# MoayedHajiAli/ElasticDiffusion-official

Measured on AMD Instinct MI355X. Metric: images/sec at 50 steps (SDXL 2048x1024), higher is better.
Workload: dtype fp16

## Files before the change

### elasticdiffusion_official_amd/csrc/gemm_kernels.hip

```cpp
#include <hip/hip_runtime.h>
#include <stdint.h>
#include <stdlib.h>

#include "elastic_hip.h"

namespace {

typedef float f32x4 __attribute__((ext_vector_type(4)));
typedef __bf16 bf16x8 __attribute__((ext_vector_type(8)));
typedef _Float16 f16x8 __attribute__((ext_vector_type(8)));
typedef uint32_t u32x4 __attribute__((ext_vector_type(4)));
typedef __attribute__((address_space(3))) void* lds_ptr_t;

struct BF {
  typedef bf16x8 v8;
  static __device__ __forceinline__ f32x4 mfma(v8 a, v8 b, f32x4 c) {
    return __builtin_amdgcn_mfma_f32_16x16x32_bf16(a, b, c, 0, 0, 0);
  }
  static __device__ __forceinline__ float to_f32(uint16_t h) { return __builtin_bit_cast(float, (uint32_t)h << 16); }
  static __device__ __forceinline__ uint16_t from_f32(float f) { return __builtin_bit_cast(uint16_t, (__bf16)f); }
  static __device__ __forceinline__ uint32_t pack2(float lo, float hi) {
    typedef float f2 __attribute__((ext_vector_type(2)));
    typedef __bf16 b2 __attribute__((ext_vector_type(2)));
    return __builtin_bit_cast(uint32_t, __builtin_convertvector(f2{lo, hi}, b2));
  }
};
struct HF {
  typedef f16x8 v8;
  static __device__ __forceinline__ f32x4 mfma(v8 a, v8 b, f32x4 c) {
    return __builtin_amdgcn_mfma_f32_16x16x32_f16(a, b, c, 0, 0, 0);
  }
  static __device__ __forceinline__ float to_f32(uint16_t h) { return (float)__builtin_bit_cast(_Float16, h); }
  static __device__ __forceinline__ uint16_t from_f32(float f) { return __builtin_bit_cast(uint16_t, (_Float16)f); }
  static __device__ __forceinline__ uint32_t pack2(float lo, float hi) {
    typedef float f2 __attribute__((ext_vector_type(2)));
    typedef _Float16 h2 __attribute__((ext_vector_type(2)));
    return __builtin_bit_cast(uint32_t, __builtin_convertvector(f2{lo, hi}, h2));
  }
};

constexpr int BM = 256;
constexpr int BN = 128;
constexpr int BK = 64;
constexpr int SUB = 1024;
constexpr int W_REGION = 32768;
constexpr int BUF = 65536;

__device__ __forceinline__ int swz(int p) { return p ^ (((p >> 9) & 1) << 5); }
__device__ __forceinline__ constexpr int x_sub(int rg, int kh) { return (rg * 2 + kh) * SUB; }
__device__ __forceinline__ constexpr int w_sub(int rg, int kh) { return W_REGION + (rg * 2 + kh) * SUB; }

__device__ __forceinline__ float gelu_as(float x) {
  const float z = __builtin_fabsf(x) * 0.70710678118654752f;
  const float t = __builtin_amdgcn_rcpf(__builtin_fmaf(0.3275911f, z, 1.0f));
  float p = __builtin_fmaf(1.061405429f, t, -1.453152027f);
  p = __builtin_fmaf(p, t, 1.421413741f);
  p = __builtin_fmaf(p, t, -0.284496736f);
  p = __builtin_fmaf(p, t, 0.254829592f);
  const float q = p * t * __builtin_amdgcn_exp2f(-1.4426950408889634f * z * z);
  const float h = 0.5f * x * q;
  return x > 0.f ? x - h : h;
}

__device__ __forceinline__ float abs_mul(float a, float b) {
  float r;
  asm("v_mul_f32_e64 %0, |%1|, %2" : "=v"(r) : "v"(a), "v"(b));
  return r;
}
__device__ __forceinline__ float relu1(float a) {
  float r;
  asm("v_max_f32_e32 %0, 0, %1" : "=v"(r) : "v"(a));
  return r;
}
__device__ __forceinline__ float geglu_one(float v, float g) {
  const float z = abs_mul(g, 0.70710678118654752f);
  const float t = __builtin_amdgcn_rcpf(__builtin_fmaf(0.3275911f, z, 1.0f));
  float p = __builtin_fmaf(0.5f * 1.061405429f, t, 0.5f * -1.453152027f);
  p = __builtin_fmaf(p, t, 0.5f * 1.421413741f);
  p = __builtin_fmaf(p, t, 0.5f * -0.284496736f);
  p = __builtin_fmaf(p, t, 0.5f * 0.254829592f);
  const float hq = (p * t) * __builtin_amdgcn_exp2f((-1.4426950408889634f * z) * z);
  return v * (relu1(g) - abs_mul(g, hq));
}

#define ED_WAIT_VM(n) asm volatile("s_waitcnt vmcnt(" #n ")" ::: "memory")
#define ED_WAIT_LGKM(n) asm volatile("s_waitcnt lgkmcnt(" #n ")" ::: "memory")
#define ED_BARRIER()                          \
  do {                                        \
    asm volatile("s_barrier" ::: "memory");   \
    __builtin_amdgcn_sched_barrier(0);        \
  } while (0)

struct Ctx {
  __amdgpu_buffer_rsrc_t xr, wr_;
  int x_voff[2], w_voff[2];
  int px_mask[2];
  int img_w, cin2, cpt;
  int wave;
  int xrd, wrd;
};

constexpr int CONV_UP2X = 2;
constexpr int CONV_S2 = 3;
constexpr int CONV_S2P0 = 4;
struct KPos {
  int tile, tap, ct, w;
};
template <int CONV>
__device__ __forceinline__ KPos k_next(KPos p, int cpt) {
  ++p.tile;
  if (CONV) {
    ++p.tap;
    p.w += cpt;
    if (p.tap == 9) {
      p.tap = 0;
      ++p.ct;
      p.w = p.ct;
    }
  } else {
    p.w = p.tile;
  }
  return p;
}

template <int BUFI, int CONV>
__device__ __forceinline__ void stage_x(uint8_t* lds, const Ctx& c, KPos p, int h) {
  const int rg = (c.wave & 3) + 8 * (c.wave >> 2) + 4 * h;
  uint8_t* dst = lds + BUFI * BUF + x_sub(0, 0) + rg * (2 * SUB);
  if (CONV) {
    const int dy = p.tap / 3 - 1, dx = p.tap - 3 * (p.tap / 3) - 1;
    int delta;
    if (CONV == CONV_UP2X) {
      const int yp = (c.px_mask[h] >> 16) & 1, xp = (c.px_mask[h] >> 17) & 1;
      delta = (((yp + dy) >> 1) * c.img_w + ((xp + dx) >> 1)) * c.cin2 + p.ct * (BK * 2);
    } else {
      delta = (dy * c.img_w + dx) * c.cin2 + p.ct * (BK * 2);
    }
    const int vo = ((c.px_mask[h] >> p.tap) & 1) ? c.x_voff[h] + delta : (int)0x80000000;
    __builtin_amdgcn_raw_ptr_buffer_load_lds(c.xr, (lds_ptr_t)dst, 16, vo, 0, 0, 0);
    __builtin_amdgcn_raw_ptr_buffer_load_lds(c.xr, (lds_ptr_t)(dst + SUB), 16, vo + 64, 0, 0, 0);
  } else {
    const int vo = c.x_voff[h] + p.tile * (BK * 2);
    __builtin_amdgcn_raw_ptr_buffer_load_lds(c.xr, (lds_ptr_t)dst, 16, vo, 0, 0, 0);
    __builtin_amdgcn_raw_ptr_buffer_load_lds(c.xr, (lds_ptr_t)(dst + SUB), 16, vo + 64, 0, 0, 0);
  }
}
template <int BUFI>
__device__ __forceinline__ void stage_w(uint8_t* lds, const Ctx& c, int widx, int g) {
  const int rg = 8 * g + c.wave;
  const int vo = c.w_voff[g] + widx * (BK * 2);
  uint8_t* dst = lds + BUFI * BUF + w_sub(0, 0) + rg * (2 * SUB);
  __builtin_amdgcn_raw_ptr_buffer_load_lds(c.wr_, (lds_ptr_t)dst, 16, vo, 0, 0, 0);
  __builtin_amdgcn_raw_ptr_buffer_load_lds(c.wr_, (lds_ptr_t)(dst + SUB), 16, vo + 64, 0, 0, 0);
}

template <class T>
struct Frags {
  typename T::v8 x[4][2];
  typename T::v8 wv[2][2];
  typename T::v8 wg[2][2];
};

template <class T, int BUFI>
__device__ __forceinline__ void read_x(const uint8_t* lds, const Ctx& c, Frags<T>& f, int mh) {
#pragma unroll
  for (int mf = 0; mf < 4; ++mf)
#pragma unroll
    for (int kh = 0; kh < 2; ++kh)
      f.x[mf][kh] = *reinterpret_cast<const typename T::v8*>(lds + c.xrd + BUFI * BUF + x_sub(mh * 4 + mf, kh));
}
template <class T, int BUFI, int G>
__device__ __forceinline__ void read_w(const uint8_t* lds, const Ctx& c, Frags<T>& f) {
#pragma unroll
  for (int nf = 0; nf < 2; ++nf)
#pragma unroll
    for (int kh = 0; kh < 2; ++kh) {
      typename T::v8 v = *reinterpret_cast<const typename T::v8*>(lds + c.wrd + BUFI * BUF + w_sub(8 * G + nf, kh) - W_REGION);
      if (G == 0) f.wv[nf][kh] = v; else f.wg[nf][kh] = v;
    }
}

template <class T, int MH, int G>
__device__ __forceinline__ void mma16(f32x4 (&acc)[8][4], const Frags<T>& f) {
  __builtin_amdgcn_s_setprio(1);
#pragma unroll
  for (int kh = 0; kh < 2; ++kh)
#pragma unroll
    for (int mf = 0; mf < 4; ++mf)
#pragma unroll
      for (int nf = 0; nf < 2; ++nf)
        acc[MH * 4 + mf][G * 2 + nf] = T::mfma(G == 0 ? f.wv[nf][kh] : f.wg[nf][kh], f.x[mf][kh], acc[MH * 4 + mf][G * 2 + nf]);
  __builtin_amdgcn_s_setprio(0);
}

template <class T, int BUFI, int CONV, bool FIRST = false>
__device__ __forceinline__ void tile_phases(uint8_t* lds, const Ctx& c, Frags<T>& f, f32x4 (&acc)[8][4], int tile, bool s1,
                                            bool s2, KPos p1, KPos p2) {
  read_w<T, BUFI, 0>(lds, c, f);
  __builtin_amdgcn_sched_barrier(0);
  read_x<T, BUFI>(lds, c, f, 0);
  if (s1) stage_x<BUFI ^ 1, CONV>(lds, c, p1, 1);
  ED_WAIT_LGKM(8);
  if (FIRST) ED_WAIT_VM(10);
  ED_BARRIER();
  ED_WAIT_LGKM(0);
  __builtin_amdgcn_sched_barrier(0);
  mma16<T, 0, 0>(acc, f);
  if (FIRST) ED_WAIT_VM(10);
  ED_BARRIER();
  read_w<T, BUFI, 1>(lds, c, f);
  if (s2) stage_w<BUFI>(lds, c, p2.w, 0);
  if (FIRST) ED_WAIT_VM(10);
  ED_BARRIER();
  ED_WAIT_LGKM(0);
  __builtin_amdgcn_sched_barrier(0);
  mma16<T, 0, 1>(acc, f);
  if (FIRST) ED_WAIT_VM(10);
  ED_BARRIER();
  read_x<T, BUFI>(lds, c, f, 1);
  if (s2) stage_x<BUFI, CONV>(lds, c, p2, 0);
  ED_BARRIER();
  ED_WAIT_LGKM(0);
  __builtin_amdgcn_sched_barrier(0);
  mma16<T, 1, 1>(acc, f);
  ED_BARRIER();
  if (s2) {
    stage_w<BUFI>(lds, c, p2.w, 1);
    ED_WAIT_VM(6);
  } else {
    ED_WAIT_VM(0);
  }
  ED_BARRIER();
  mma16<T, 1, 0>(acc, f);
  ED_BARRIER();
}

constexpr int TWO_MIN_TILES = 20;
template <class T, int BUFI, int CONV>
__device__ __forceinline__ void tile_phases_two(uint8_t* lds, const Ctx& c, Frags<T>& f, f32x4 (&acc)[8][4], int tile, bool s1, bool s2,
                                                KPos p1, KPos p2) {
  read_w<T, BUFI, 0>(lds, c, f);
  read_x<T, BUFI>(lds, c, f, 0);
  read_w<T, BUFI, 1>(lds, c, f);
  if (s1) stage_x<BUFI ^ 1, CONV>(lds, c, p1, 1);
  ED_WAIT_LGKM(0);
  ED_BARRIER();
  mma16<T, 0, 0>(acc, f);
  mma16<T, 0, 1>(acc, f);
  ED_BARRIER();
  read_x<T, BUFI>(lds, c, f, 1);
  if (s2) {
    stage_w<BUFI>(lds, c, p2.w, 0);
    stage_x<BUFI, CONV>(lds, c, p2, 0);
    stage_w<BUFI>(lds, c, p2.w, 1);
    ED_WAIT_VM(6);
  } else {
    ED_WAIT_VM(0);
  }
  ED_WAIT_LGKM(0);
  ED_BARRIER();
  mma16<T, 1, 1>(acc, f);
  mma16<T, 1, 0>(acc, f);
  ED_BARRIER();
}

template <class T, int BUFI, int CONV>
__device__ __forceinline__ void tile_phases_half(uint8_t* lds, const Ctx& c, Frags<T>& f, f32x4 (&acc)[8][4], int tile, bool s1, bool s2,
                                                 KPos p1, KPos p2) {
  read_w<T, BUFI, 0>(lds, c, f);
  read_x<T, BUFI>(lds, c, f, 0);
  if (s1) stage_x<BUFI ^ 1, CONV>(lds, c, p1, 1);
  ED_WAIT_LGKM(0);
  ED_BARRIER();
  mma16<T, 0, 0>(acc, f);
  ED_BARRIER();
  read_x<T, BUFI>(lds, c, f, 1);
  if (s2) {
    stage_w<BUFI>(lds, c, p2.w, 0);
    stage_x<BUFI, CONV>(lds, c, p2, 0);
    ED_WAIT_VM(4);
  } else {
    ED_WAIT_VM(0);
  }
  ED_WAIT_LGKM(0);
  ED_BARRIER();
  mma16<T, 1, 0>(acc, f);
  ED_BARRIER();
}

template <class T, int BUFI, int CONV>
__device__ __forceinline__ void tile_phases_rows(uint8_t* lds, const Ctx& c, Frags<T>& f, f32x4 (&acc)[8][4], bool s1, bool s2, KPos p1,
                                                 KPos p2) {
  read_w<T, BUFI, 0>(lds, c, f);
  read_x<T, BUFI>(lds, c, f, 0);
  if (s1) stage_w<BUFI ^ 1>(lds, c, p1.w, 1);
  ED_WAIT_LGKM(0);
  ED_BARRIER();
  mma16<T, 0, 0>(acc, f);
  ED_BARRIER();
  read_w<T, BUFI, 1>(lds, c, f);
  if (s2) {
    stage_w<BUFI>(lds, c, p2.w, 0);
    stage_x<BUFI, CONV>(lds, c, p2, 0);
    ED_WAIT_VM(4);
  } else {
    ED_WAIT_VM(0);
  }
  ED_WAIT_LGKM(0);
  ED_BARRIER();
  mma16<T, 0, 1>(acc, f);
  ED_BARRIER();
}

template <class T, int EPI, int CONV, bool ADD = true, bool OUT32 = false, bool TWO = false, bool ROWS = false>
__global__ void __launch_bounds__(512, 2)
k_gemm_8phase(const uint16_t* __restrict__ x, const uint16_t* __restrict__ w, const uint16_t* __restrict__ bias,
              const uint16_t* __restrict__ row_bias, const uint16_t* __restrict__ residual, uint16_t* __restrict__ out, int M,
              int K, int I, int n_blocks_n, int n_blocks, int img_h, int img_w, int rows_per_sample, float out_scale,
              const float* __restrict__ act_absmax) {
  __shared__ __attribute__((aligned(1024))) uint8_t lds[2 * BUF];

  const int bid = blockIdx.x;
  const int q = n_blocks >> 3, r = n_blocks & 7, xcd = bid & 7;
  const int tid = (xcd < r ? xcd * (q + 1) : r * (q + 1) + (xcd - r) * q) + (bid >> 3);
  const int n_blocks_m = n_blocks / n_blocks_n;
  const int per_group = 8 * n_blocks_n, grp = tid / per_group, first = grp * 8;
  const int rows_here = n_blocks_m - first < 8 ? n_blocks_m - first : 8;
  constexpr int TBM = ROWS ? BM / 2 : BM;
  constexpr int WROWS = TBM / 2;
  constexpr int NMB = WROWS / 16;
  const int m0 = (first + (tid % per_group) % rows_here) * TBM;
  const int n0 = ((tid % per_group) / rows_here) * (EPI == 0 ? BN : 2 * BN);
  const int gap = EPI == 0 ? I : BN;

  const int lane = threadIdx.x & 63;
  Ctx c;
  c.wave = __builtin_amdgcn_readfirstlane(threadIdx.x >> 6);
  const int wrow = c.wave >> 2, wcol = c.wave & 3;

  const int ps = swz(16 * lane), srow = ps >> 6, skb = ps & 63;
  const int row_bytes = K * 2;
  const int x_row_bytes = CONV ? row_bytes / 9 : row_bytes;
  c.xr = __builtin_amdgcn_make_buffer_rsrc((void*)x, 0, (int)((int64_t)(CONV == CONV_UP2X ? M / 4 : CONV >= CONV_S2 ? 4 * (int64_t)M : M) * x_row_bytes),
                                           0x00020000);
  c.wr_ = __builtin_amdgcn_make_buffer_rsrc((void*)w, 0, (int)((int64_t)(EPI == 0 ? 2 : 1) * I * row_bytes), 0x00020000);
  const int xrow0 = m0 + ((c.wave & 3) + (ROWS ? 4 : 8) * (c.wave >> 2)) * 16 + srow;
  c.x_voff[0] = xrow0 * x_row_bytes + skb;
  c.x_voff[1] = c.x_voff[0] + 64 * x_row_bytes;
  c.img_w = CONV == CONV_UP2X ? img_w / 2 : CONV >= CONV_S2 ? 2 * img_w : img_w;
  c.cin2 = x_row_bytes;
  c.cpt = CONV ? K / (9 * BK) : 1;
  c.px_mask[0] = c.px_mask[1] = 0;
  if (CONV) {
#pragma unroll
    for (int h = 0; h < 2; ++h) {
      const int m = xrow0 + 64 * h;
      if (m < M) {
        const int rem = m % (img_h * img_w), py = rem / img_w, px = rem - py * img_w;
        int mask = 0;
#pragma unroll
        for (int t = 0; t < 9; ++t) {
          if (CONV == CONV_S2) {
            if (2 * py + t / 3 - 1 >= 0 && 2 * px + t % 3 - 1 >= 0) mask |= 1 << t;
          } else if (CONV == CONV_S2P0) {
            if (2 * py + t / 3 < 2 * img_h && 2 * px + t % 3 < 2 * img_w) mask |= 1 << t;
          } else {
            const int yy = py + t / 3 - 1, xx = px + t % 3 - 1;
            if (yy >= 0 && yy < img_h && xx >= 0 && xx < img_w) mask |= 1 << t;
          }
        }
        c.px_mask[h] = mask;
        if (CONV == CONV_UP2X) {
          const int hs = img_h / 2, ws = img_w / 2;
          c.px_mask[h] = mask | ((py & 1) << 16) | ((px & 1) << 17);
          c.x_voff[h] = ((m / (img_h * img_w)) * (hs * ws) + (py >> 1) * ws + (px >> 1)) * x_row_bytes + skb;
        }
        if (CONV >= CONV_S2) {
          const int o1 = CONV == CONV_S2P0 ? 1 : 0;
          c.x_voff[h] = (((m / (img_h * img_w)) * (2 * img_h) + 2 * py + o1) * (2 * img_w) + 2 * px + o1) * x_row_bytes + skb;
        }
      }
    }
  }
  c.w_voff[0] = (n0 + 32 * (c.wave >> 1) + 8 * (srow >> 2) + (srow & 3) + 4 * (c.wave & 1)) * row_bytes + skb;
  c.w_voff[1] = c.w_voff[0] + gap * row_bytes;
  const int rd = swz((lane & 15) * 64 + (lane >> 4) * 16);
  c.xrd = rd + wrow * 8 * (2 * SUB);
  c.wrd = rd + W_REGION + wcol * 2 * (2 * SUB);

  const int ncol = n0 + 32 * wcol + 8 * (lane >> 4);
  u32x4 bias_v = {0, 0, 0, 0}, bias_g = {0, 0, 0, 0};
  if (bias && !OUT32) {
    if (EPI == 0 || ncol < I) bias_v = *reinterpret_cast<const u32x4*>(bias + ncol);
    if (EPI == 0 || ncol + gap < I) bias_g = *reinterpret_cast<const u32x4*>(bias + gap + ncol);
  }

  f32x4 acc[8][4];
#pragma unroll
  for (int a = 0; a < 8; ++a)
#pragma unroll
    for (int b = 0; b < 4; ++b) acc[a][b] = f32x4{0.f, 0.f, 0.f, 0.f};
  Frags<T> f;

  const int nt = K / BK;
  const KPos p0 = {0, 0, 0, 0};
  KPos pa = k_next<CONV>(p0, c.cpt);
  KPos pb = k_next<CONV>(pa, c.cpt);
  const bool half = !ROWS && EPI == 1 && n0 + BN >= I;
  if (ROWS) {
    stage_w<0>(lds, c, 0, 0);
    stage_x<0, CONV>(lds, c, p0, 0);
    stage_w<0>(lds, c, 0, 1);
    if (nt > 1) {
      stage_w<1>(lds, c, pa.w, 0);
      stage_x<1, CONV>(lds, c, pa, 0);
      ED_WAIT_VM(4);
    } else {
      ED_WAIT_VM(0);
    }
    ED_BARRIER();
    if (wrow == 1) ED_BARRIER();
    int tr = 0;
    for (; tr + 1 < nt; tr += 2) {
      tile_phases_rows<T, 0, CONV>(lds, c, f, acc, true, tr + 2 < nt, pa, pb);
      pa = pb;
      pb = k_next<CONV>(pb, c.cpt);
      tile_phases_rows<T, 1, CONV>(lds, c, f, acc, tr + 2 < nt, tr + 3 < nt, pa, pb);
      pa = pb;
      pb = k_next<CONV>(pb, c.cpt);
    }
    if (tr < nt) tile_phases_rows<T, 0, CONV>(lds, c, f, acc, false, false, pa, pb);
    if (wrow == 0) ED_BARRIER();
  } else if (half) {
    stage_w<0>(lds, c, 0, 0);
    stage_x<0, CONV>(lds, c, p0, 0);
    stage_x<0, CONV>(lds, c, p0, 1);
    if (nt > 1) {
      stage_w<1>(lds, c, pa.w, 0);
      stage_x<1, CONV>(lds, c, pa, 0);
      ED_WAIT_VM(4);
    } else {
      ED_WAIT_VM(0);
    }
    ED_BARRIER();
    if (wrow == 1) ED_BARRIER();
    int th = 0;
    for (; th + 1 < nt; th += 2) {
      tile_phases_half<T, 0, CONV>(lds, c, f, acc, th, true, th + 2 < nt, pa, pb);
      pa = pb;
      pb = k_next<CONV>(pb, c.cpt);
      tile_phases_half<T, 1, CONV>(lds, c, f, acc, th + 1, th + 2 < nt, th + 3 < nt, pa, pb);
      pa = pb;
      pb = k_next<CONV>(pb, c.cpt);
    }
    if (th < nt) tile_phases_half<T, 0, CONV>(lds, c, f, acc, th, false, false, pa, pb);
    if (wrow == 0) ED_BARRIER();
  } else {
  stage_w<0>(lds, c, 0, 0);
  stage_x<0, CONV>(lds, c, p0, 0);
  stage_w<0>(lds, c, 0, 1);
  stage_x<0, CONV>(lds, c, p0, 1);
  constexpr bool two = TWO;
  const bool early = nt >= 3 && !two;
  if (nt > 1) {
    stage_w<1>(lds, c, pa.w, 0);
    stage_x<1, CONV>(lds, c, pa, 0);
    stage_w<1>(lds, c, pa.w, 1);
    if (early) ED_WAIT_VM(10);
    else ED_WAIT_VM(6);
  } else {
    ED_WAIT_VM(0);
  }
  ED_BARRIER();
  if (wrow == 1) ED_BARRIER();

  int t = 0;
  if (two) {
    for (; t + 1 < nt; t += 2) {
      tile_phases_two<T, 0, CONV>(lds, c, f, acc, t, true, t + 2 < nt, pa, pb);
      pa = pb;
      pb = k_next<CONV>(pb, c.cpt);
      tile_phases_two<T, 1, CONV>(lds, c, f, acc, t + 1, t + 2 < nt, t + 3 < nt, pa, pb);
      pa = pb;
      pb = k_next<CONV>(pb, c.cpt);
    }
    if (t < nt) tile_phases_two<T, 0, CONV>(lds, c, f, acc, t, false, false, pa, pb);
    t = nt;
  }
  if (early) {
    tile_phases<T, 0, CONV, true>(lds, c, f, acc, 0, true, true, pa, pb);
    pa = pb;
    pb = k_next<CONV>(pb, c.cpt);
    tile_phases<T, 1, CONV>(lds, c, f, acc, 1, true, 3 < nt, pa, pb);
    pa = pb;
    pb = k_next<CONV>(pb, c.cpt);
    t = 2;
  }
  for (; t + 1 < nt; t += 2) {
    tile_phases<T, 0, CONV>(lds, c, f, acc, t, true, t + 2 < nt, pa, pb);
    pa = pb;
    pb = k_next<CONV>(pb, c.cpt);
    tile_phases<T, 1, CONV>(lds, c, f, acc, t + 1, t + 2 < nt, t + 3 < nt, pa, pb);
    pa = pb;
    pb = k_next<CONV>(pb, c.cpt);
  }
  if (t < nt) tile_phases<T, 0, CONV>(lds, c, f, acc, t, false, false, pa, pb);
  if (wrow == 0) ED_BARRIER();
  }

  if (OUT32) {
    const float* biasf = reinterpret_cast<const float*>(bias);
    const float* resf = reinterpret_cast<const float*>(residual);
    float* outf = reinterpret_cast<float*>(out);
    if (act_absmax) {
      const int E = (int)((__builtin_bit_cast(uint32_t, *act_absmax) >> 23) & 0xffu) - 127;
      const int e = E > 14 ? E - 14 : 0;
      out_scale *= __builtin_bit_cast(float, (uint32_t)(127 + e) << 23);
    }
    const bool col_v = ncol < I, col_g = ncol + gap < I;
    f32x4 b32[2][2] = {{f32x4{0.f, 0.f, 0.f, 0.f}, f32x4{0.f, 0.f, 0.f, 0.f}}, {f32x4{0.f, 0.f, 0.f, 0.f}, f32x4{0.f, 0.f, 0.f, 0.f}}};
    if (biasf) {
#pragma unroll
      for (int fr = 0; fr < 2; ++fr) {
        if (col_v) b32[0][fr] = *reinterpret_cast<const f32x4*>(biasf + ncol + 4 * fr);
        if (col_g) b32[1][fr] = *reinterpret_cast<const f32x4*>(biasf + ncol + gap + 4 * fr);
      }
    }
#pragma unroll
    for (int mb = 0; mb < NMB; ++mb) {
      const int m = m0 + WROWS * wrow + 16 * mb + (lane & 15);
      if (m >= M) continue;
#pragma unroll
      for (int hf = 0; hf < 2; ++hf) {
        if (!(hf == 0 ? col_v : col_g)) continue;
        const int64_t o = (int64_t)m * I + ncol + hf * gap;
#pragma unroll
        for (int fr = 0; fr < 2; ++fr) {
          f32x4 v = acc[mb][2 * hf + fr] * out_scale + b32[hf][fr];
          if (ADD && resf) v += *reinterpret_cast<const f32x4*>(resf + o + 4 * fr);
          *reinterpret_cast<f32x4*>(outf + o + 4 * fr) = v;
        }
      }
    }
    return;
  }
  float bv[2][4], bg[2][4];
#pragma unroll
  for (int e = 0; e < 8; ++e) {
    bv[e >> 2][e & 3] = T::to_f32((uint16_t)(bias_v[e >> 1] >> (16 * (e & 1))));
    bg[e >> 2][e & 3] = T::to_f32((uint16_t)(bias_g[e >> 1] >> (16 * (e & 1))));
  }
#pragma unroll
  for (int mb = 0; mb < NMB; ++mb) {
    const int m = m0 + WROWS * wrow + 16 * mb + (lane & 15);
    if (EPI == 0) {
      uint32_t pk[4];
#pragma unroll
      for (int nf = 0; nf < 2; ++nf)
#pragma unroll
        for (int jj = 0; jj < 2; ++jj) {
          const float o0 = geglu_one(acc[mb][nf][2 * jj] + bv[nf][2 * jj], acc[mb][2 + nf][2 * jj] + bg[nf][2 * jj]);
          const float o1 = geglu_one(acc[mb][nf][2 * jj + 1] + bv[nf][2 * jj + 1], acc[mb][2 + nf][2 * jj + 1] + bg[nf][2 * jj + 1]);
          pk[nf * 2 + jj] = T::pack2(o0, o1);
        }
      if (m < M) *reinterpret_cast<u32x4*>(out + (int64_t)m * I + ncol) = u32x4{pk[0], pk[1], pk[2], pk[3]};
    } else {
      const bool ok_v = m < M && ncol < I, ok_g = m < M && ncol + gap < I;
      u32x4 av[2] = {u32x4{0, 0, 0, 0}, u32x4{0, 0, 0, 0}}, ag[2] = {u32x4{0, 0, 0, 0}, u32x4{0, 0, 0, 0}};
      if (ADD && row_bias) {
        const int64_t rb = (int64_t)(m / rows_per_sample) * I;
        if (ok_v) av[0] = *reinterpret_cast<const u32x4*>(row_bias + rb + ncol);
        if (ok_g) ag[0] = *reinterpret_cast<const u32x4*>(row_bias + rb + ncol + gap);
      }
      if (ADD && residual) {
        if (ok_v) av[1] = *reinterpret_cast<const u32x4*>(residual + (int64_t)m * I + ncol);
        if (ok_g) ag[1] = *reinterpret_cast<const u32x4*>(residual + (int64_t)m * I + ncol + gap);
      }
      uint32_t pv[4], pg[4];
#pragma unroll
      for (int e = 0; e < 8; e += 2) {
        float v0 = acc[mb][e >> 2][e & 3] + bv[e >> 2][e & 3], v1 = acc[mb][e >> 2][(e & 3) + 1] + bv[e >> 2][(e & 3) + 1];
        float g0 = acc[mb][2 + (e >> 2)][e & 3] + bg[e >> 2][e & 3], g1 = acc[mb][2 + (e >> 2)][(e & 3) + 1] + bg[e >> 2][(e & 3) + 1];
        if (ADD) {
#pragma unroll
          for (int a = 0; a < 2; ++a) {
            v0 += T::to_f32((uint16_t)av[a][e >> 1]), v1 += T::to_f32((uint16_t)(av[a][e >> 1] >> 16));
            g0 += T::to_f32((uint16_t)ag[a][e >> 1]), g1 += T::to_f32((uint16_t)(ag[a][e >> 1] >> 16));
          }
        }
        pv[e >> 1] = (uint32_t)T::from_f32(v0) | ((uint32_t)T::from_f32(v1) << 16);
        pg[e >> 1] = (uint32_t)T::from_f32(g0) | ((uint32_t)T::from_f32(g1) << 16);
      }
      if (ok_v) *reinterpret_cast<u32x4*>(out + (int64_t)m * I + ncol) = u32x4{pv[0], pv[1], pv[2], pv[3]};
      if (ok_g) *reinterpret_cast<u32x4*>(out + (int64_t)m * I + ncol + gap) = u32x4{pg[0], pg[1], pg[2], pg[3]};
    }
  }
}

struct TilePos {
  int m0, n0;
};
__device__ __forceinline__ TilePos geglu_tile_of(int bid, int n_blocks, int n_blocks_n) {
  const int q = n_blocks >> 3, r = n_blocks & 7, xcd = bid & 7;
  const int tid = (xcd < r ? xcd * (q + 1) : r * (q + 1) + (xcd - r) * q) + (bid >> 3);
  const int n_blocks_m = n_blocks / n_blocks_n;
  const int per_group = 8 * n_blocks_n, grp = tid / per_group, first = grp * 8;
  const int rows_here = n_blocks_m - first < 8 ? n_blocks_m - first : 8;
  return TilePos{(first + (tid % per_group) % rows_here) * BM, ((tid % per_group) / rows_here) * BN};
}

template <class T>
__global__ void __launch_bounds__(512, 2)
k_geglu_persist(const uint16_t* __restrict__ x, const uint16_t* __restrict__ w, const uint16_t* __restrict__ bias,
                uint16_t* __restrict__ out, int M, int K, int I, int n_blocks_n, int n_blocks) {
  __shared__ __attribute__((aligned(1024))) uint8_t lds[2 * BUF];
  const int lane = threadIdx.x & 63;
  const int wave = __builtin_amdgcn_readfirstlane(threadIdx.x >> 6);
  const int wrow = wave >> 2, wcol = wave & 3;
  const int ps = swz(16 * lane), srow = ps >> 6, skb = ps & 63;
  const int row_bytes = K * 2;
  const int rd = swz((lane & 15) * 64 + (lane >> 4) * 16);
  const int nt = K / BK;
  const bool early = nt >= 3;

  auto setup = [&](TilePos tp) {
    Ctx c;
    c.wave = wave;
    c.xr = __builtin_amdgcn_make_buffer_rsrc((void*)x, 0, (int)((int64_t)M * row_bytes), 0x00020000);
    c.wr_ = __builtin_amdgcn_make_buffer_rsrc((void*)w, 0, (int)((int64_t)2 * I * row_bytes), 0x00020000);
    c.x_voff[0] = (tp.m0 + ((wave & 3) + 8 * (wave >> 2)) * 16 + srow) * row_bytes + skb;
    c.x_voff[1] = c.x_voff[0] + 64 * row_bytes;
    c.img_w = 0, c.cin2 = row_bytes, c.cpt = 1;
    c.px_mask[0] = c.px_mask[1] = 0;
    c.w_voff[0] = (tp.n0 + 32 * (wave >> 1) + 8 * (srow >> 2) + (srow & 3) + 4 * (wave & 1)) * row_bytes + skb;
    c.w_voff[1] = c.w_voff[0] + I * row_bytes;
    c.xrd = rd + wrow * 8 * (2 * SUB);
    c.wrd = rd + W_REGION + wcol * 2 * (2 * SUB);
    return c;
  };
  auto load_bias = [&](int ncol, u32x4& bv_raw, u32x4& bg_raw) {
    bv_raw = u32x4{0, 0, 0, 0}, bg_raw = u32x4{0, 0, 0, 0};
    if (bias) {
      bv_raw = *reinterpret_cast<const u32x4*>(bias + ncol);
      bg_raw = *reinterpret_cast<const u32x4*>(bias + I + ncol);
    }
  };
  auto issue_prologue = [&](const Ctx& c) {
    const KPos p0 = {0, 0, 0, 0}, p1 = {1, 0, 0, 1};
    stage_w<0>(lds, c, 0, 0);
    stage_x<0, false>(lds, c, p0, 0);
    stage_w<0>(lds, c, 0, 1);
    stage_x<0, false>(lds, c, p0, 1);
    if (nt > 1) {
      stage_w<1>(lds, c, 1, 0);
      stage_x<1, false>(lds, c, p1, 0);
      stage_w<1>(lds, c, 1, 1);
    }
  };

  int bid = blockIdx.x;
  TilePos tp = geglu_tile_of(bid, n_blocks, n_blocks_n);
  Ctx c = setup(tp);
  u32x4 bias_v, bias_g;
  load_bias(tp.n0 + 32 * wcol + 8 * (lane >> 4), bias_v, bias_g);
  issue_prologue(c);

  for (;;) {
    f32x4 acc[8][4];
#pragma unroll
    for (int a = 0; a < 8; ++a)
#pragma unroll
      for (int b = 0; b < 4; ++b) acc[a][b] = f32x4{0.f, 0.f, 0.f, 0.f};
    Frags<T> f;
    KPos pa = {1, 0, 0, 1}, pb = {2, 0, 0, 2};
    if (nt > 1) {
      if (early) ED_WAIT_VM(10);
      else ED_WAIT_VM(6);
    } else {
      ED_WAIT_VM(0);
    }
    ED_BARRIER();
    if (wrow == 1) ED_BARRIER();

    int t = 0;
    if (early) {
      tile_phases<T, 0, false, true>(lds, c, f, acc, 0, true, true, pa, pb);
      pa = pb, pb = KPos{pb.tile + 1, 0, 0, pb.tile + 1};
      tile_phases<T, 1, false>(lds, c, f, acc, 1, true, 3 < nt, pa, pb);
      pa = pb, pb = KPos{pb.tile + 1, 0, 0, pb.tile + 1};
      t = 2;
    }
    for (; t + 1 < nt; t += 2) {
      tile_phases<T, 0, false>(lds, c, f, acc, t, true, t + 2 < nt, pa, pb);
      pa = pb, pb = KPos{pb.tile + 1, 0, 0, pb.tile + 1};
      tile_phases<T, 1, false>(lds, c, f, acc, t + 1, t + 2 < nt, t + 3 < nt, pa, pb);
      pa = pb, pb = KPos{pb.tile + 1, 0, 0, pb.tile + 1};
    }
    if (t < nt) tile_phases<T, 0, false>(lds, c, f, acc, t, false, false, pa, pb);
    if (wrow == 0) ED_BARRIER();

    const int m0 = tp.m0, ncol = tp.n0 + 32 * wcol + 8 * (lane >> 4);
    float bv[2][4], bg[2][4];
#pragma unroll
    for (int e = 0; e < 8; ++e) {
      bv[e >> 2][e & 3] = T::to_f32((uint16_t)(bias_v[e >> 1] >> (16 * (e & 1))));
      bg[e >> 2][e & 3] = T::to_f32((uint16_t)(bias_g[e >> 1] >> (16 * (e & 1))));
    }
#pragma unroll
    for (int e = 0; e < 8; ++e) asm volatile("" : "+v"(bv[e >> 2][e & 3]), "+v"(bg[e >> 2][e & 3]));

    const int next = bid + (int)gridDim.x;
    const bool has_next = next < n_blocks;
    Ctx c2 = c;
    TilePos tp2 = tp;
    if (has_next) {
      tp2 = geglu_tile_of(next, n_blocks, n_blocks_n);
      c2 = setup(tp2);
      load_bias(tp2.n0 + 32 * wcol + 8 * (lane >> 4), bias_v, bias_g);
      __builtin_amdgcn_sched_barrier(0);
      issue_prologue(c2);
      __builtin_amdgcn_sched_barrier(0);
    }
#pragma unroll
    for (int mb = 0; mb < 8; ++mb) {
      const int m = m0 + 128 * wrow + 16 * mb + (lane & 15);
      uint32_t pk[4];
#pragma unroll
      for (int nf = 0; nf < 2; ++nf)
#pragma unroll
        for (int jj = 0; jj < 2; ++jj) {
          const float o0 = geglu_one(acc[mb][nf][2 * jj] + bv[nf][2 * jj], acc[mb][2 + nf][2 * jj] + bg[nf][2 * jj]);
          const float o1 = geglu_one(acc[mb][nf][2 * jj + 1] + bv[nf][2 * jj + 1], acc[mb][2 + nf][2 * jj + 1] + bg[nf][2 * jj + 1]);
          pk[nf * 2 + jj] = T::pack2(o0, o1);
        }
      if (m < M) *reinterpret_cast<u32x4*>(out + (int64_t)m * I + ncol) = u32x4{pk[0], pk[1], pk[2], pk[3]};
    }
    if (!has_next) break;
    bid = next, tp = tp2, c = c2;
  }
}

}

static int gemm_cus() {
  static int cus[16] = {0};
  int dev = 0;
  if (hipGetDevice(&dev) != hipSuccess || dev < 0 || dev >= 16) return 0;
  if (cus[dev] == 0) {
    int n = 0;
    if (hipDeviceGetAttribute(&n, hipDeviceAttributeMultiprocessorCount, dev) != hipSuccess || n < 8) return 0;
    cus[dev] = n / 8 * 8;
  }
  return cus[dev];
}
constexpr double ROWS_TILE_COST = 0.72;

template <int EPI, int CONV, bool OUT32 = false>
static int launch(const void* x, const void* w, const void* bias, const void* row_bias, const void* residual, void* out, int dtype,
                  int64_t M, int K, int I, int img_h, int img_w, int rows_per_sample, void* stream, float out_scale = 1.0f,
                  const float* act_absmax = nullptr) {
  if (M == 0) return 0;
  const int bad = (int)hipErrorInvalidValue;
  if (M < 0 || K % BK != 0 || K < BK || I <= 0 || (EPI == 0 ? I % BN != 0 : I % 8 != 0)) return bad;
  if (CONV && (K % (9 * BK) != 0 || img_h <= 0 || img_w <= 0 || M % ((int64_t)img_h * img_w) != 0)) return bad;
  if (CONV == CONV_UP2X && (img_h % 2 != 0 || img_w % 2 != 0 || row_bias || residual)) return bad;
  if (CONV >= CONV_S2 && (row_bias || residual || 4 * M * (int64_t)(K / 9) * 2 >= 0x7ffffff0ll)) return bad;
  if (row_bias && (rows_per_sample <= 0 || M % rows_per_sample != 0)) return bad;
  if (M * (int64_t)(CONV ? K / 9 : K) * 2 >= 0x7ffffff0ll || (int64_t)(EPI == 0 ? 2 : 1) * I * K * 2 >= 0x7ffffff0ll) return bad;
  if ((((uintptr_t)x | (uintptr_t)w | (uintptr_t)out | (uintptr_t)bias | (uintptr_t)row_bias | (uintptr_t)residual) & 15u)) return bad;
  const int nbn = EPI == 0 ? I / BN : (I + 2 * BN - 1) / (2 * BN);
  const int64_t nb256 = ((M + BM - 1) / BM) * nbn, nb128 = ((M + BM / 2 - 1) / (BM / 2)) * nbn;
  if (nb128 >= (1ll << 31) || M >= (1ll << 31)) return bad;
  hipStream_t s = (hipStream_t)stream;
  const bool add = EPI == 1 && (row_bias || residual);
  const bool two = CONV && K / BK >= TWO_MIN_TILES;
  bool rows = false;
  if (!OUT32 && EPI == 1 && CONV < CONV_UP2X) {
    const int cus = gemm_cus();
    const double r256 = (double)((nb256 + cus - 1) / cus), r128 = (double)((nb128 + cus - 1) / cus) * ROWS_TILE_COST;
    rows = cus > 0 && r128 < r256 - 1e-9;
    if (const char* e = getenv("ED_GEMM_ROWS")) rows = e[0] == '1' ? true : (e[0] == '0' ? false : rows);
  }
  const int64_t nb = rows ? nb128 : nb256;
#define ED_LAUNCH1(TT, ADD_, TWO_, ROWS_)                                                                                            \
  k_gemm_8phase<TT, EPI, CONV, ADD_, OUT32, TWO_, ROWS_><<<(int)nb, 512, 0, s>>>((const uint16_t*)x, (const uint16_t*)w, (const uint16_t*)bias, \
                                                             (const uint16_t*)row_bias, (const uint16_t*)residual, (uint16_t*)out,  \
                                                             (int)M, K, I, nbn, (int)nb, img_h, img_w, rows_per_sample > 0 ? rows_per_sample : 1, out_scale, \
                                                             act_absmax)
#define ED_LAUNCH(TT, ADD_)                                   \
  do {                                                        \
    if constexpr (OUT32 || EPI == 0) {                        \
      if constexpr (CONV) {                                   \
        if (two) ED_LAUNCH1(TT, ADD_, true, false);           \
        else ED_LAUNCH1(TT, ADD_, false, false);              \
      } else {                                                \
        ED_LAUNCH1(TT, ADD_, false, false);                   \
      }                                                       \
    } else if (CONV < CONV_UP2X && rows) {                    \
      if constexpr (CONV < CONV_UP2X) ED_LAUNCH1(TT, ADD_, false, true);   \
    } else if constexpr (CONV) {                              \
      if (two) ED_LAUNCH1(TT, ADD_, true, false);             \
      else ED_LAUNCH1(TT, ADD_, false, false);                \
    } else {                                                  \
      ED_LAUNCH1(TT, ADD_, false, false);                     \
    }                                                         \
  } while (0)
  if constexpr (OUT32) {
    if (dtype != ED_F16 || row_bias) return bad;
    if constexpr (CONV >= CONV_UP2X) {
      ED_LAUNCH(HF, false);
    } else {
      if (add) ED_LAUNCH(HF, true);
      else ED_LAUNCH(HF, false);
    }
  } else {
    if constexpr (CONV >= CONV_UP2X) {
      if (dtype == ED_BF16) ED_LAUNCH(BF, false);
      else if (dtype == ED_F16) ED_LAUNCH(HF, false);
      else return bad;
    } else if (dtype == ED_BF16) {
      if (EPI == 0 || add) ED_LAUNCH(BF, true);
      else ED_LAUNCH(BF, EPI == 0);
    } else if (dtype == ED_F16) {
      if (EPI == 0 || add) ED_LAUNCH(HF, true);
      else ED_LAUNCH(HF, EPI == 0);
    } else {
      return bad;
    }
  }
#undef ED_LAUNCH
#undef ED_LAUNCH1
  return (int)hipGetLastError();
}

extern "C" {

int ed_geglu_gemm(const void* x, const void* w, const void* bias, void* out, int dtype, int64_t M, int K, int I, void* stream) {
  if (M == 0) return 0;
  const int bad = (int)hipErrorInvalidValue;
  if (M < 0 || K % BK != 0 || K < BK || I <= 0 || I % BN != 0) return bad;
  if (M * (int64_t)K * 2 >= 0x7ffffff0ll || (int64_t)2 * I * K * 2 >= 0x7ffffff0ll) return bad;
  if ((((uintptr_t)x | (uintptr_t)w | (uintptr_t)out | (uintptr_t)bias) & 15u)) return bad;
  const int nbn = I / BN;
  const int64_t nb = ((M + BM - 1) / BM) * nbn;
  if (nb >= (1ll << 31) || M >= (1ll << 31)) return bad;
  const int ncu = gemm_cus();
  if (ncu <= 0) return (int)hipErrorInvalidDevice;
  const int grid = nb < ncu ? (int)nb : ncu;
  hipStream_t s = (hipStream_t)stream;
  if (dtype == ED_BF16)
    k_geglu_persist<BF><<<grid, 512, 0, s>>>((const uint16_t*)x, (const uint16_t*)w, (const uint16_t*)bias, (uint16_t*)out, (int)M, K, I, nbn, (int)nb);
  else if (dtype == ED_F16)
    k_geglu_persist<HF><<<grid, 512, 0, s>>>((const uint16_t*)x, (const uint16_t*)w, (const uint16_t*)bias, (uint16_t*)out, (int)M, K, I, nbn, (int)nb);
  else
    return bad;
  return (int)hipGetLastError();
}

int ed_linear(const void* x, const void* w, const void* bias, const void* residual, void* out, int dtype, int64_t M, int K, int N,
              void* stream) {
  return launch<1, 0>(x, w, bias, nullptr, residual, out, dtype, M, K, N, 0, 0, 0, stream);
}

int ed_conv3x3_nhwc(const void* x, const void* w, const void* bias, const void* sample_bias, const void* residual, void* out,
                    int dtype, int B, int H, int W, int Cin, int N, void* stream) {
  if (B < 0 || H <= 0 || W <= 0 || Cin <= 0) return (int)hipErrorInvalidValue;
  return launch<1, 1>(x, w, bias, sample_bias, residual, out, dtype, (int64_t)B * H * W, 9 * Cin, N, H, W, H * W, stream);
}

int ed_conv3x3_nhwc_up2x(const void* x, const void* w, const void* bias, void* out, int dtype, int B, int H, int W, int Cin, int N,
                         void* stream) {
  if (B < 0 || H <= 0 || W <= 0 || Cin <= 0) return (int)hipErrorInvalidValue;
  if ((int64_t)B * (H / 2) * (W / 2) * Cin * 2 >= 0x7ffffff0ll) return (int)hipErrorInvalidValue;
  return launch<1, CONV_UP2X>(x, w, bias, nullptr, nullptr, out, dtype, (int64_t)B * H * W, 9 * Cin, N, H, W, H * W, stream);
}

int ed_conv3x3_nhwc_s2(const void* x, const void* w, const void* bias, void* out, int dtype, int B, int H, int W, int Cin, int N,
                       void* stream) {
  if (B < 0 || H <= 0 || W <= 0 || Cin <= 0) return (int)hipErrorInvalidValue;
  return launch<1, CONV_S2>(x, w, bias, nullptr, nullptr, out, dtype, (int64_t)B * H * W, 9 * Cin, N, H, W, H * W, stream);
}

int ed_conv3x3_nhwc_f32out(const void* x, const void* w, const float* bias, const float* residual, float* out, int dtype, int B, int H, int W,
                           int Cin, int N, float out_scale, const float* act_absmax, void* stream) {
  if (B < 0 || H <= 0 || W <= 0 || Cin <= 0 || ((uintptr_t)act_absmax & 3u)) return (int)hipErrorInvalidValue;
  return launch<1, 1, true>(x, w, bias, nullptr, residual, out, dtype, (int64_t)B * H * W, 9 * Cin, N, H, W, H * W, stream, out_scale,
                               act_absmax);
}

int ed_conv3x3_nhwc_f32out_s2(const void* x, const void* w, const float* bias, float* out, int dtype, int B, int H, int W, int Cin, int N,
                              float out_scale, const float* act_absmax, void* stream) {
  if (B < 0 || H <= 0 || W <= 0 || Cin <= 0 || ((uintptr_t)act_absmax & 3u)) return (int)hipErrorInvalidValue;
  return launch<1, CONV_S2P0, true>(x, w, bias, nullptr, nullptr, out, dtype, (int64_t)B * H * W, 9 * Cin, N, H, W, H * W, stream, out_scale,
                                    act_absmax);
}

}
```

Baseline: 0.1020.

## Add persistent tile-walking projection GEMM that overlaps next-tile prologue with epilogue

Adds a persistent kernel for projection-style GEMMs (EPI==1, non-rows path) that launches one block per CU and walks several output tiles per block. While the current tile's epilogue stores run, it issues the next tile's context setup, bias loads and LDS prologue, hiding per-tile launch and pipeline fill cost. It is enabled by default whenever there are more tiles than the grid, with env overrides for grid size and enablement. The trade-offs are higher register pressure, a fixed XCD-aware tile order that may balance worse than hardware scheduling, and a much larger device code path.

New measurement: 0.1017. No clear change (-0.4%).

```diff
diff --git a/elasticdiffusion_official_amd/csrc/gemm_kernels.hip b/elasticdiffusion_official_amd/csrc/gemm_kernels.hip
--- a/elasticdiffusion_official_amd/csrc/gemm_kernels.hip
+++ b/elasticdiffusion_official_amd/csrc/gemm_kernels.hip
@@ -312,30 +312,94 @@
   ED_BARRIER();
 }
 
-template <class T, int EPI, int CONV, bool ADD = true, bool OUT32 = false, bool TWO = false, bool ROWS = false>
-__global__ void __launch_bounds__(512, 2)
-k_gemm_8phase(const uint16_t* __restrict__ x, const uint16_t* __restrict__ w, const uint16_t* __restrict__ bias,
-              const uint16_t* __restrict__ row_bias, const uint16_t* __restrict__ residual, uint16_t* __restrict__ out, int M,
-              int K, int I, int n_blocks_n, int n_blocks, int img_h, int img_w, int rows_per_sample, float out_scale,
-              const float* __restrict__ act_absmax) {
-  __shared__ __attribute__((aligned(1024))) uint8_t lds[2 * BUF];
-
-  const int bid = blockIdx.x;
-  const int q = n_blocks >> 3, r = n_blocks & 7, xcd = bid & 7;
-  const int tid = (xcd < r ? xcd * (q + 1) : r * (q + 1) + (xcd - r) * q) + (bid >> 3);
-  const int n_blocks_m = n_blocks / n_blocks_n;
-  const int per_group = 8 * n_blocks_n, grp = tid / per_group, first = grp * 8;
-  const int rows_here = n_blocks_m - first < 8 ? n_blocks_m - first : 8;
-  constexpr int TBM = ROWS ? BM / 2 : BM;
-  constexpr int WROWS = TBM / 2;
-  constexpr int NMB = WROWS / 16;
-  const int m0 = (first + (tid % per_group) % rows_here) * TBM;
-  const int n0 = ((tid % per_group) / rows_here) * (EPI == 0 ? BN : 2 * BN);
-  const int gap = EPI == 0 ? I : BN;
-
-  const int lane = threadIdx.x & 63;
+template <int CONV>
+__device__ __forceinline__ void issue_prologue(uint8_t* lds, const Ctx& c, int nt, bool half) {
+  const KPos p0 = {0, 0, 0, 0};
+  const KPos pa = k_next<CONV>(p0, c.cpt);
+  stage_w<0>(lds, c, 0, 0);
+  stage_x<0, CONV>(lds, c, p0, 0);
+  if (!half) stage_w<0>(lds, c, 0, 1);
+  stage_x<0, CONV>(lds, c, p0, 1);
+  if (nt > 1) {
+    stage_w<1>(lds, c, pa.w, 0);
+    stage_x<1, CONV>(lds, c, pa, 0);
+    if (!half) stage_w<1>(lds, c, pa.w, 1);
+  }
+}
+
+template <class T, int CONV, bool TWO>
+__device__ __forceinline__ void k_loop(uint8_t* lds, const Ctx& c, Frags<T>& f, f32x4 (&acc)[8][4], int nt, bool half) {
+  const int wrow = c.wave >> 2;
+  KPos pa = k_next<CONV>(KPos{0, 0, 0, 0}, c.cpt);
+  KPos pb = k_next<CONV>(pa, c.cpt);
+  if (half) {
+    if (nt > 1) ED_WAIT_VM(4);
+    else ED_WAIT_VM(0);
+    ED_BARRIER();
+    if (wrow == 1) ED_BARRIER();
+    int th = 0;
+    for (; th + 1 < nt; th += 2) {
+      tile_phases_half<T, 0, CONV>(lds, c, f, acc, th, true, th + 2 < nt, pa, pb);
+      pa = pb;
+      pb = k_next<CONV>(pb, c.cpt);
+      tile_phases_half<T, 1, CONV>(lds, c, f, acc, th + 1, th + 2 < nt, th + 3 < nt, pa, pb);
+      pa = pb;
+      pb = k_next<CONV>(pb, c.cpt);
+    }
+    if (th < nt) tile_phases_half<T, 0, CONV>(lds, c, f, acc, th, false, false, pa, pb);
+    if (wrow == 0) ED_BARRIER();
+    return;
+  }
+  constexpr bool two = TWO;
+  const bool early = nt >= 3 && !two;
+  if (nt > 1) {
+    if (early) ED_WAIT_VM(10);
+    else ED_WAIT_VM(6);
+  } else {
+    ED_WAIT_VM(0);
+  }
+  ED_BARRIER();
+  if (wrow == 1) ED_BARRIER();
+
+  int t = 0;
+  if (two) {
+    for (; t + 1 < nt; t += 2) {
+      tile_phases_two<T, 0, CONV>(lds, c, f, acc, t, true, t + 2 < nt, pa, pb);
+      pa = pb;
+      pb = k_next<CONV>(pb, c.cpt);
+      tile_phases_two<T, 1, CONV>(lds, c, f, acc, t + 1, t + 2 < nt, t + 3 < nt, pa, pb);
+      pa = pb;
+      pb = k_next<CONV>(pb, c.cpt);
+    }
+    if (t < nt) tile_phases_two<T, 0, CONV>(lds, c, f, acc, t, false, false, pa, pb);
+    t = nt;
+  }
+  if (early) {
+    tile_phases<T, 0, CONV, true>(lds, c, f, acc, 0, true, true, pa, pb);
+    pa = pb;
+    pb = k_next<CONV>(pb, c.cpt);
+    tile_phases<T, 1, CONV>(lds, c, f, acc, 1, true, 3 < nt, pa, pb);
+    pa = pb;
+    pb = k_next<CONV>(pb, c.cpt);
+    t = 2;
+  }
+  for (; t + 1 < nt; t += 2) {
+    tile_phases<T, 0, CONV>(lds, c, f, acc, t, true, t + 2 < nt, pa, pb);
+    pa = pb;
+    pb = k_next<CONV>(pb, c.cpt);
+    tile_phases<T, 1, CONV>(lds, c, f, acc, t + 1, t + 2 < nt, t + 3 < nt, pa, pb);
+    pa = pb;
+    pb = k_next<CONV>(pb, c.cpt);
+  }
+  if (t < nt) tile_phases<T, 0, CONV>(lds, c, f, acc, t, false, false, pa, pb);
+  if (wrow == 0) ED_BARRIER();
+}
+
+template <int EPI, int CONV, bool ROWS>
+__device__ __forceinline__ Ctx make_ctx(const uint16_t* x, const uint16_t* w, int M, int K, int I, int img_h, int img_w, int m0, int n0,
+                                        int gap, int wave, int lane) {
   Ctx c;
-  c.wave = __builtin_amdgcn_readfirstlane(threadIdx.x >> 6);
+  c.wave = wave;
   const int wrow = c.wave >> 2, wcol = c.wave & 3;
 
   const int ps = swz(16 * lane), srow = ps >> 6, skb = ps & 63;
@@ -387,6 +451,118 @@
   const int rd = swz((lane & 15) * 64 + (lane >> 4) * 16);
   c.xrd = rd + wrow * 8 * (2 * SUB);
   c.wrd = rd + W_REGION + wcol * 2 * (2 * SUB);
+  return c;
+}
+
+template <class T, bool ADD>
+__device__ __forceinline__ void proj_store_row(const f32x4 (&acc)[4], const float (&bv)[2][4], const float (&bg)[2][4],
+                                               const uint16_t* __restrict__ row_bias, const uint16_t* __restrict__ residual,
+                                               uint16_t* __restrict__ out, int m, int M, int I, int ncol, int gap, int rows_per_sample) {
+  const bool ok_v = m < M && ncol < I, ok_g = m < M && ncol + gap < I;
+  u32x4 av[2] = {u32x4{0, 0, 0, 0}, u32x4{0, 0, 0, 0}}, ag[2] = {u32x4{0, 0, 0, 0}, u32x4{0, 0, 0, 0}};
+  if (ADD && row_bias) {
+    const int64_t rb = (int64_t)(m / rows_per_sample) * I;
+    if (ok_v) av[0] = *reinterpret_cast<const u32x4*>(row_bias + rb + ncol);
+    if (ok_g) ag[0] = *reinterpret_cast<const u32x4*>(row_bias + rb + ncol + gap);
+  }
+  if (ADD && residual) {
+    if (ok_v) av[1] = *reinterpret_cast<const u32x4*>(residual + (int64_t)m * I + ncol);
+    if (ok_g) ag[1] = *reinterpret_cast<const u32x4*>(residual + (int64_t)m * I + ncol + gap);
+  }
+  uint32_t pv[4], pg[4];
+#pragma unroll
+  for (int e = 0; e < 8; e += 2) {
+    float v0 = acc[e >> 2][e & 3] + bv[e >> 2][e & 3], v1 = acc[e >> 2][(e & 3) + 1] + bv[e >> 2][(e & 3) + 1];
+    float g0 = acc[2 + (e >> 2)][e & 3] + bg[e >> 2][e & 3], g1 = acc[2 + (e >> 2)][(e & 3) + 1] + bg[e >> 2][(e & 3) + 1];
+    if (ADD) {
+#pragma unroll
+      for (int a = 0; a < 2; ++a) {
+        v0 += T::to_f32((uint16_t)av[a][e >> 1]), v1 += T::to_f32((uint16_t)(av[a][e >> 1] >> 16));
+        g0 += T::to_f32((uint16_t)ag[a][e >> 1]), g1 += T::to_f32((uint16_t)(ag[a][e >> 1] >> 16));
+      }
+    }
+    pv[e >> 1] = (uint32_t)T::from_f32(v0) | ((uint32_t)T::from_f32(v1) << 16);
+    pg[e >> 1] = (uint32_t)T::from_f32(g0) | ((uint32_t)T::from_f32(g1) << 16);
+  }
+  if (ok_v) *reinterpret_cast<u32x4*>(out + (int64_t)m * I + ncol) = u32x4{pv[0], pv[1], pv[2], pv[3]};
+  if (ok_g) *reinterpret_cast<u32x4*>(out + (int64_t)m * I + ncol + gap) = u32x4{pg[0], pg[1], pg[2], pg[3]};
+}
+
+template <class T, int EPI, int CONV, bool ADD = true, bool OUT32 = false, bool TWO = false, bool ROWS = false>
+__global__ void __launch_bounds__(512, 2)
+k_gemm_8phase(const uint16_t* __restrict__ x, const uint16_t* __restrict__ w, const uint16_t* __restrict__ bias,
+              const uint16_t* __restrict__ row_bias, const uint16_t* __restrict__ residual, uint16_t* __restrict__ out, int M,
+              int K, int I, int n_blocks_n, int n_blocks, int img_h, int img_w, int rows_per_sample, float out_scale,
+              const float* __restrict__ act_absmax) {
+  __shared__ __attribute__((aligned(1024))) uint8_t lds[2 * BUF];
+
+  const int bid = blockIdx.x;
+  const int q = n_blocks >> 3, r = n_blocks & 7, xcd = bid & 7;
+  const int tid = (xcd < r ? xcd * (q + 1) : r * (q + 1) + (xcd - r) * q) + (bid >> 3);
+  const int n_blocks_m = n_blocks / n_blocks_n;
+  const int per_group = 8 * n_blocks_n, grp = tid / per_group, first = grp * 8;
+  const int rows_here = n_blocks_m - first < 8 ? n_blocks_m - first : 8;
+  constexpr int TBM = ROWS ? BM / 2 : BM;
+  constexpr int WROWS = TBM / 2;
+  constexpr int NMB = WROWS / 16;
+  const int m0 = (first + (tid % per_group) % rows_here) * TBM;
+  const int n0 = ((tid % per_group) / rows_here) * (EPI == 0 ? BN : 2 * BN);
+  const int gap = EPI == 0 ? I : BN;
+
+  const int lane = threadIdx.x & 63;
+  Ctx c;
+  c.wave = __builtin_amdgcn_readfirstlane(threadIdx.x >> 6);
+  const int wrow = c.wave >> 2, wcol = c.wave & 3;
+
+  const int ps = swz(16 * lane), srow = ps >> 6, skb = ps & 63;
+  const int row_bytes = K * 2;
+  const int x_row_bytes = CONV ? row_bytes / 9 : row_bytes;
+  c.xr = __builtin_amdgcn_make_buffer_rsrc((void*)x, 0, (int)((int64_t)(CONV == CONV_UP2X ? M / 4 : CONV >= CONV_S2 ? 4 * (int64_t)M : M) * x_row_bytes),
+                                           0x00020000);
+  c.wr_ = __builtin_amdgcn_make_buffer_rsrc((void*)w, 0, (int)((int64_t)(EPI == 0 ? 2 : 1) * I * row_bytes), 0x00020000);
+  const int xrow0 = m0 + ((c.wave & 3) + (ROWS ? 4 : 8) * (c.wave >> 2)) * 16 + srow;
+  c.x_voff[0] = xrow0 * x_row_bytes + skb;
+  c.x_voff[1] = c.x_voff[0] + 64 * x_row_bytes;
+  c.img_w = CONV == CONV_UP2X ? img_w / 2 : CONV >= CONV_S2 ? 2 * img_w : img_w;
+  c.cin2 = x_row_bytes;
+  c.cpt = CONV ? K / (9 * BK) : 1;
+  c.px_mask[0] = c.px_mask[1] = 0;
+  if (CONV) {
+#pragma unroll
+    for (int h = 0; h < 2; ++h) {
+      const int m = xrow0 + 64 * h;
+      if (m < M) {
+        const int rem = m % (img_h * img_w), py = rem / img_w, px = rem - py * img_w;
+        int mask = 0;
+#pragma unroll
+        for (int t = 0; t < 9; ++t) {
+          if (CONV == CONV_S2) {
+            if (2 * py + t / 3 - 1 >= 0 && 2 * px + t % 3 - 1 >= 0) mask |= 1 << t;
+          } else if (CONV == CONV_S2P0) {
+            if (2 * py + t / 3 < 2 * img_h && 2 * px + t % 3 < 2 * img_w) mask |= 1 << t;
+          } else {
+            const int yy = py + t / 3 - 1, xx = px + t % 3 - 1;
+            if (yy >= 0 && yy < img_h && xx >= 0 && xx < img_w) mask |= 1 << t;
+          }
+        }
+        c.px_mask[h] = mask;
+        if (CONV == CONV_UP2X) {
+          const int hs = img_h / 2, ws = img_w / 2;
+          c.px_mask[h] = mask | ((py & 1) << 16) | ((px & 1) << 17);
+          c.x_voff[h] = ((m / (img_h * img_w)) * (hs * ws) + (py >> 1) * ws + (px >> 1)) * x_row_bytes + skb;
+        }
+        if (CONV >= CONV_S2) {
+          const int o1 = CONV == CONV_S2P0 ? 1 : 0;
+          c.x_voff[h] = (((m / (img_h * img_w)) * (2 * img_h) + 2 * py + o1) * (2 * img_w) + 2 * px + o1) * x_row_bytes + skb;
+        }
+      }
+    }
+  }
+  c.w_voff[0] = (n0 + 32 * (c.wave >> 1) + 8 * (srow >> 2) + (srow & 3) + 4 * (c.wave & 1)) * row_bytes + skb;
+  c.w_voff[1] = c.w_voff[0] + gap * row_bytes;
+  const int rd = swz((lane & 15) * 64 + (lane >> 4) * 16);
+  c.xrd = rd + wrow * 8 * (2 * SUB);
+  c.wrd = rd + W_REGION + wcol * 2 * (2 * SUB);
 
   const int ncol = n0 + 32 * wcol + 8 * (lane >> 4);
   u32x4 bias_v = {0, 0, 0, 0}, bias_g = {0, 0, 0, 0};
@@ -740,6 +916,96 @@
   }
 }
 
+__device__ __forceinline__ bool walk_tile(int b, int G, int k, int n_blocks, int n_blocks_n, TilePos& tp) {
+  const int q = n_blocks >> 3, r = n_blocks & 7, xcd = b & 7, g = G >> 3;
+  const int local = ((b >> 3) + 8 * k) % g + g * k;
+  if (local >= q + (xcd < r ? 1 : 0)) return false;
+  const int tid = (xcd < r ? xcd * (q + 1) : r * (q + 1) + (xcd - r) * q) + local;
+  const int n_blocks_m = n_blocks / n_blocks_n;
+  const int per_group = 8 * n_blocks_n, grp = tid / per_group, first = grp * 8;
+  const int rows_here = n_blocks_m - first < 8 ? n_blocks_m - first : 8;
+  tp = TilePos{(first + (tid % per_group) % rows_here) * BM, ((tid % per_group) / rows_here) * (2 * BN)};
+  return true;
+}
+
+template <class T, int CONV, bool ADD, bool TWO>
+__global__ void __launch_bounds__(512, 2)
+k_proj_walk(const uint16_t* __restrict__ x, const uint16_t* __restrict__ w, const uint16_t* __restrict__ bias,
+            const uint16_t* __restrict__ row_bias, const uint16_t* __restrict__ residual, uint16_t* __restrict__ out, int M, int K, int I,
+            int n_blocks_n, int n_blocks, int img_h, int img_w, int rows_per_sample) {
+  __shared__ __attribute__((aligned(1024))) uint8_t lds[2 * BUF];
+  auto lane_id = [&] {
+    int l = threadIdx.x & 63;
+    asm volatile("" : "+v"(l));
+    return l;
+  };
+  auto fresh = [](int v) {
+    asm volatile("" : "+s"(v));
+    return v;
+  };
+  int lane = lane_id();
+  const int wave = __builtin_amdgcn_readfirstlane(threadIdx.x >> 6);
+  const int wrow = wave >> 2, wcol = wave & 3;
+  const int nt = K / BK;
+  const int b = blockIdx.x, G = gridDim.x;
+
+  auto load_bias = [&](int ncol, u32x4& bv_raw, u32x4& bg_raw) {
+    bv_raw = u32x4{0, 0, 0, 0}, bg_raw = u32x4{0, 0, 0, 0};
+    if (bias) {
+      if (ncol < I) bv_raw = *reinterpret_cast<const u32x4*>(bias + ncol);
+      if (ncol + BN < I) bg_raw = *reinterpret_cast<const u32x4*>(bias + BN + ncol);
+    }
+  };
+
+  TilePos tp = {0, 0};
+  walk_tile(b, G, 0, n_blocks, n_blocks_n, tp);
+  Ctx c = make_ctx<1, CONV, false>(x, w, M, K, I, fresh(img_h), fresh(img_w), tp.m0, tp.n0, BN, wave, lane);
+  bool half = tp.n0 + BN >= I;
+  u32x4 bias_v, bias_g;
+  load_bias(tp.n0 + 32 * wcol + 8 * (lane >> 4), bias_v, bias_g);
+  issue_prologue<CONV>(lds, c, nt, half);
+
+  for (int k = 1;; ++k) {
+    f32x4 acc[8][4];
+#pragma unroll
+    for (int a = 0; a < 8; ++a)
+#pragma unroll
+      for (int e = 0; e < 4; ++e) acc[a][e] = f32x4{0.f, 0.f, 0.f, 0.f};
+    Frags<T> f;
+    TilePos tp2 = tp;
+    const bool has_next = walk_tile(b, G, k, n_blocks, n_blocks_n, tp2);
+    k_loop<T, CONV, TWO>(lds, c, f, acc, nt, half);
+
+    lane = lane_id();
+    const int m0 = tp.m0, ncol = tp.n0 + 32 * wcol + 8 * (lane >> 4);
+    float bv[2][4], bg[2][4];
+#pragma unroll
+    for (int e = 0; e < 8; ++e) {
+      bv[e >> 2][e & 3] = T::to_f32((uint16_t)(bias_v[e >> 1] >> (16 * (e & 1))));
+      bg[e >> 2][e & 3] = T::to_f32((uint16_t)(bias_g[e >> 1] >> (16 * (e & 1))));
+    }
+#pragma unroll
+    for (int e = 0; e < 8; ++e) asm volatile("" : "+v"(bv[e >> 2][e & 3]), "+v"(bg[e >> 2][e & 3]));
+
+    Ctx c2 = c;
+    bool half2 = half;
+    if (has_next) {
+      c2 = make_ctx<1, CONV, false>(x, w, M, K, I, fresh(img_h), fresh(img_w), tp2.m0, tp2.n0, BN, wave, lane);
+      half2 = tp2.n0 + BN >= I;
+      load_bias(tp2.n0 + 32 * wcol + 8 * (lane >> 4), bias_v, bias_g);
+      __builtin_amdgcn_sched_barrier(0);
+      issue_prologue<CONV>(lds, c2, nt, half2);
+      __builtin_amdgcn_sched_barrier(0);
+    }
+    const int rps = fresh(rows_per_sample);
+#pragma unroll
+    for (int mb = 0; mb < 8; ++mb)
+      proj_store_row<T, ADD>(acc[mb], bv, bg, row_bias, residual, out, m0 + 128 * wrow + 16 * mb + (lane & 15), M, I, ncol, BN, rps);
+    if (!has_next) break;
+    tp = tp2, c = c2, half = half2;
+  }
+}
+
 }
 
 static int gemm_cus() {
@@ -753,6 +1019,7 @@
   }
   return cus[dev];
 }
+constexpr bool WALK_DEFAULT = true;
 constexpr double ROWS_TILE_COST = 0.72;
 
 template <int EPI, int CONV, bool OUT32 = false>
@@ -777,9 +1044,25 @@
   bool rows = false;
   if (!OUT32 && EPI == 1 && CONV < CONV_UP2X) {
     const int cus = gemm_cus();
+    if (cus <= 0) return (int)hipErrorInvalidDevice;
     const double r256 = (double)((nb256 + cus - 1) / cus), r128 = (double)((nb128 + cus - 1) / cus) * ROWS_TILE_COST;
-    rows = cus > 0 && r128 < r256 - 1e-9;
+    rows = r128 < r256 - 1e-9;
     if (const char* e = getenv("ED_GEMM_ROWS")) rows = e[0] == '1' ? true : (e[0] == '0' ? false : rows);
+  }
+  int walk_grid = 0;
+  if constexpr (!OUT32 && EPI == 1 && CONV <= CONV_UP2X) {
+    if (!rows) {
+      const int cus = gemm_cus();
+      if (cus <= 0) return (int)hipErrorInvalidDevice;
+      int grid = cus;
+      if (const char* e = getenv("ED_GEMM_PERSIST_GRID")) {
+        const int cap = atoi(e) / 8 * 8;
+        if (cap >= 8 && cap < grid) grid = cap;
+      }
+      bool walk = WALK_DEFAULT;
+      if (const char* e = getenv("ED_GEMM_PERSIST")) walk = e[0] == '1' ? true : (e[0] == '0' ? false : walk);
+      if (walk && nb256 > grid) walk_grid = grid;
+    }
   }
   const int64_t nb = rows ? nb128 : nb256;
 #define ED_LAUNCH1(TT, ADD_, TWO_, ROWS_)                                                                                            \
@@ -787,8 +1070,23 @@
                                                              (const uint16_t*)row_bias, (const uint16_t*)residual, (uint16_t*)out,  \
                                                              (int)M, K, I, nbn, (int)nb, img_h, img_w, rows_per_sample > 0 ? rows_per_sample : 1, out_scale, \
                                                              act_absmax)
+#define ED_LAUNCHW(TT, ADD_, TWO_)                                                                                                  \
+  k_proj_walk<TT, CONV, ADD_, TWO_><<<walk_grid, 512, 0, s>>>((const uint16_t*)x, (const uint16_t*)w, (const uint16_t*)bias,                \
+                                                              (const uint16_t*)row_bias, (const uint16_t*)residual, (uint16_t*)out, (int)M, \
+                                                              K, I, nbn, (int)nb, img_h, img_w, rows_per_sample > 0 ? rows_per_sample : 1)
 #define ED_LAUNCH(TT, ADD_)                                   \
   do {                                                        \
+    if constexpr (!OUT32 && EPI == 1 && CONV <= CONV_UP2X) {  \
+      if (walk_grid) {                                        \
+        if constexpr (CONV) {                                 \
+          if (two) ED_LAUNCHW(TT, ADD_, true);                \
+          else ED_LAUNCHW(TT, ADD_, false);                   \
+        } else {                                              \
+          ED_LAUNCHW(TT, ADD_, false);                        \
+        }                                                     \
+        break;                                                \
+      }                                                       \
+    }                                                         \
     if constexpr (OUT32 || EPI == 0) {                        \
       if constexpr (CONV) {                                   \
         if (two) ED_LAUNCH1(TT, ADD_, true, false);           \
@@ -829,6 +1127,7 @@
     }
   }
 #undef ED_LAUNCH
+#undef ED_LAUNCHW
 #undef ED_LAUNCH1
   return (int)hipGetLastError();
 }
```
